# rhysnewell/Lorikeet

Hardware: AMD Instinct MI355X
Metric: PairHMM cell-updates/s (GCUPS) (higher is better)
Workload: dtype f64; 1 GPU; config2 x 1024 regions per GPU: 128 reads x 8 haps, R=150, H=300; regions_per_gpu=1024, seed=1000, env=PHMM_REGION_OWN_QUEUE=0 in this process only

## Files before the change

lorikeet_amd/csrc/phmm_chain_kernels.hip:

```cpp
#include "phmm_device.hpp"

namespace phmm {

namespace {

#ifndef PHMM_CHAIN_L
#define PHMM_CHAIN_L 16
#endif
constexpr int CL = PHMM_CHAIN_L;
#ifndef PHMM_RING
#define PHMM_RING 256
#endif
constexpr int RING = PHMM_RING;
constexpr int RING_SLOTS = RING + 4 + 1;
constexpr int CHAIN_META = CHAIN_MAX_READS + 8;
constexpr uint32_t X_PAD = 0x100u;
constexpr uint32_t X_NONE = 0x102u;
constexpr int LEAD = CL - 1;

__device__ __forceinline__ double from_left_inject(double v, double inject, bool group_head) {
    constexpr int ctrl = CL == 16 ? 0x111 : 0x138;
    int lo = __builtin_amdgcn_update_dpp(__double2loint(inject), __double2loint(v), ctrl, 0xf, 0xf, false);
    int hi = __builtin_amdgcn_update_dpp(__double2hiint(inject), __double2hiint(v), ctrl, 0xf, 0xf, false);
    if constexpr (CL == 32) {
        lo = group_head ? __double2loint(inject) : lo;
        hi = group_head ? __double2hiint(inject) : hi;
    }
    return __hiloint2double(hi, lo);
}

__device__ __forceinline__ RowConst row_bytes_one_go(const ForwardParams &p, uint32_t x, uint32_t q, uint32_t q_prev, uint32_t iq,
                                                     uint32_t dq, uint32_t dq_prev, uint32_t g, uint32_t g_next, bool first,
                                                     bool last) {
    const uint32_t mx = max(iq, dq), mn = min(iq, dq);
    const double mi = p.eps[iq], ii = p.eps[g], mm = p.mm[((mx * (mx + 1)) >> 1) + mn];
    const double e_g_next = p.eps[g_next], e_q_prev = p.eps[q_prev], e_dq_prev = p.eps[dq_prev];
    const double inv_om = p.inv_om[g], ratio_mis = p.ratio_mis[q];
    RowConst n;
    n.dd = ii;
    const double im = 1.0 - ii;
    const double im_next = last ? 1.0 : 1.0 - e_g_next;
    const double pm_prev = first ? 1.0 : 1.0 - e_q_prev;
    n.mm = mm * pm_prev;
    n.bI = mi * im_next * pm_prev;
    n.gI = ii * (im_next * inv_om);
    n.dDp = first ? 1.0 : e_dq_prev * im * pm_prev;
    n.pm = 1.0;
    n.px = (x == 'N') ? 1.0 : ratio_mis;
    n.x = x;
    n.pad0 = 0;
    n.pad1 = 0.0;
    return n;
}

template <int K>
__device__ __forceinline__ void chain_fallback(const ForwardParams &p, const ChainItem &it, RowConst *ring, int lane,
                                               int grp, int l, const HapCols<K> &hc, int H, bool hv, int a, int Nh) {
    const uint32_t reg = it.region;
    for (uint32_t r = it.read_begin; r < it.read_end; ++r) {
        const uint32_t ro = p.read_off[r];
        const int R = (int)(p.read_off[r + 1] - ro);
        bool z = false;
        for (int row = lane; row < R; row += WAVE) z |= row_blocks_prescale(p, ro + row);
        const bool scaled = __ballot(z) == 0ull;
        const bool staged = R + 1 <= RING;
        lds_wave_sync();
        if (staged) {
            if (lane == 0) ring[0] = neutral_row();
            for (int row = lane; row < R; row += WAVE) ring[row + 1] = make_row(p, ro, row, R, scaled);
        }
        lds_wave_sync();
        const double scale0 = (scaled && R > 0) ? 1.0 - p.eps[p.gcp[ro]] : 1.0;
        const double fin = (scaled && R > 0) ? 1.0 - p.eps[p.base_q[ro + R - 1]] : 1.0;
        const double c0 = p.initial_condition / (double)H * scale0;
        const bool group_head = (CL == 32) && (lane == 32);
        double s = staged ? sweep_general<CL, K>(LdsView{ring}, R, l, group_head, hc, H, c0, scaled, fin)
                          : sweep_general<CL, K>(GlobalRowView{p, ro, R, scaled}, R, l, group_head, hc, H, c0, scaled, fin);
#pragma unroll
        for (int off = CL / 2; off > 0; off >>= 1) s += __shfl_xor(s, off, WAVE);
        if (l == 0 && hv) {
            const double v = log10(s) - p.initial_condition_log10;
            p.out[p.out_off[reg] + (uint64_t)(r - p.region_read_off[reg]) * (uint64_t)Nh + a] = v;
            if (const uint32_t sb = status_bits(v)) atomicOr(p.status, sb);
        }
    }
    (void)grp;
}

template <int K>
__device__ __forceinline__ void chain_fallback_streams(const ForwardParams &p, uint32_t reg, uint32_t r_begin, int n_mine,
                                                       int n_iter, int lane, int l, const HapCols<K> &hc, int H, bool hv,
                                                       int a, int Nh) {
    const uint64_t group_bits = 0xffffull << (lane & ~15);
    for (int i = 0; i < n_iter; ++i) {
        const bool valid = i < n_mine;
        const uint32_t r = r_begin + (uint32_t)i;
        const uint32_t ro = valid ? p.read_off[r] : 0u;
        const int R = valid ? (int)(p.read_off[r + 1] - ro) : 0;
        bool z = false;
        for (int row = l; row < R; row += 16) z |= row_blocks_prescale(p, ro + row);
        const bool scaled = (__ballot(z) & group_bits) == 0ull;
        const double scale0 = (scaled && R > 0) ? 1.0 - p.eps[p.gcp[ro]] : 1.0;
        const double fin = (scaled && R > 0) ? 1.0 - p.eps[p.base_q[ro + R - 1]] : 1.0;
        const double c0 = p.initial_condition / (double)H * scale0;
        double s = sweep_general<16, K>(GlobalRowView{p, ro, R, scaled}, R, l, false, hc, H, c0, scaled, fin);
#pragma unroll
        for (int off = 8; off > 0; off >>= 1) s += __shfl_xor(s, off, WAVE);
        if (l == 0 && hv && valid) {
            const double v = log10(s) - p.initial_condition_log10;
            p.out[p.out_off[reg] + (uint64_t)(r - p.region_read_off[reg]) * (uint64_t)Nh + a] = v;
            if (const uint32_t sb = status_bits(v)) atomicOr(p.status, sb);
        }
    }
}

}

template <int CLT, int K, int MODE = CHAIN_PLAIN>
__device__ __forceinline__ void chain_body(const ForwardParams &p, const ChainItem it, unsigned char *smem, const ChainItemX *x = nullptr,
                                           double *park = nullptr) {
    static_assert(CLT == CL, "one lanes-per-pair value per compilation unit");
    static_assert(MODE == CHAIN_PLAIN || CL == 16, "prefix sharing: 16 lanes per pair");
    const int col0 = MODE == CHAIN_SUFFIX ? (int)x->mask_or_col0 : 0;
    const uint32_t park_rows = MODE == CHAIN_PLAIN ? 0u : 16u * x->park_rows16;
    const uint32_t park_mask = MODE == CHAIN_PARK ? (uint32_t)x->mask_or_col0 : 0u;
    const int lane = threadIdx.x;
    const int grp = lane / CL, l = lane % CL;
    const bool group_head = (CL == 32) && (lane == 32);
    const uint32_t reg = it.region;
    const int n_chain = (int)(it.read_end - it.read_begin);
    const uint32_t h0 = p.region_hap_off[reg];
    const int Nh = (int)(p.region_hap_off[reg + 1] - h0);
    const int S = (CL == 16) ? (int)it.streams : 1;
    const int GS = (WAVE / CL) / S;
    const int sid = grp / GS;
    const int a = MODE == CHAIN_PLAIN ? (int)it.quad * GS + grp % GS : (int)x->hap[grp & 3];
    const bool hv = a < Nh;
    const int n_sub = (n_chain + S - 1) / S;
    const int TPS = (RING / 4) / S;
    const int NM = RING / S - 1;
    auto n_of = [&](int s) { return max(0, min(n_sub, n_chain - s * n_sub)); };
    const int n_mine = n_of(sid);
    uint32_t ho = 0;
    int H = 0;
    if (hv) {
        ho = p.hap_off[h0 + a];
        H = (int)(p.hap_off[h0 + a + 1] - ho);
    }
    RowConst *ring = reinterpret_cast<RowConst *>(smem);
    uint32_t *roff = reinterpret_cast<uint32_t *>(ring + RING_SLOTS);
    uint32_t *stot = roff + CHAIN_META;

    HapCols<K> hc;
    bool lane_n = false;
#pragma unroll
    for (int w = 0; w < HapCols<K>::W; ++w) hc.y[w] = 0u;
#pragma unroll
    for (int k = 0; k < K; ++k) {
        const int col = col0 + l * K + k;
        uint32_t y = col < H ? (uint32_t)p.hap_bases[ho + col] : X_PAD;
        const bool is_n = (y == 'N');
        lane_n |= is_n;
        hc.set(k, y);
    }

    const uint32_t rb = it.read_begin;
    const uint32_t byte0 = p.read_off[rb];
    const uint32_t bytes = p.read_off[it.read_end] - byte0;
    const bool z = chain_blocks_prescale(p, byte0, bytes, lane);
    if ((__ballot(z) | __ballot(lane_n)) != 0ull) {
        if constexpr (MODE == CHAIN_SUFFIX) {
            for (uint32_t r = rb + (uint32_t)l; r < it.read_end && hv; r += CL)
                p.out[p.out_off[reg] + (uint64_t)(r - p.region_read_off[reg]) * (uint64_t)Nh + a] = __longlong_as_double(0x7ff8000000000000ll);
            if (lane == 0) atomicOr(p.status, STATUS_RESCUE);
            return;
        }
        if (S == 1)
            chain_fallback<K>(p, it, ring, lane, grp, l, hc, H, hv, a, Nh);
        else if constexpr (CL == 16)
            chain_fallback_streams<K>(p, reg, rb + (uint32_t)(sid * n_sub), n_mine, n_sub, lane, l, hc, H, hv, a, Nh);
        return;
    }
    {
        const int sj = lane / n_sub, ij = lane % n_sub;
        uint32_t len = lane < n_chain ? p.read_off[rb + lane + 1] - p.read_off[rb + lane] + 2u : 0u;
        uint32_t incl = len;
#pragma unroll
        for (int off = 1; off < WAVE; off <<= 1) {
            const uint32_t v = __shfl_up(incl, off, WAVE);
            if (lane >= off) incl += v;
        }
        const uint32_t before = __shfl(incl, max(sj * n_sub - 1, 0), WAVE);
        const int cb = sj * (n_sub + 1);
        if (lane < 4) stot[lane] = 0u;
        if (lane < n_chain) {
            roff[cb + ij] = p.read_off[rb + lane];
            if (ij + 1 == n_of(sj)) {
                roff[cb + ij + 1] = p.read_off[rb + lane + 1];
                stot[sj] = incl - (sj > 0 ? before : 0u);
            }
        }
        if (lane == 0) ring[RING_SLOTS - 1] = neutral_row();
    }
    lds_wave_sync();
    const int S_max = (int)max(max(stot[0], stot[1]), max(stot[2], stot[3]));
    const double c_unit = ldexp(1.0, 1010);

    uint32_t pb_x = 0, pb_q = 0, pb_qp = 0, pb_i = 0, pb_d = 0, pb_dp = 0, pb_g = 0, pb_gn = 0;
    double pb_bM = 0.0, pb_bD = 0.0;
    int p_Q = 0;
    const bool producer = lane < S * TPS;
    const int ps = producer ? lane / TPS : 0, pj = lane % TPS;
    const int pcb = ps * (n_sub + 1), pn = n_of(ps);
    int p_lo = 0, p_row = pj - LEAD - TPS;
    p_Q = pj - TPS;
    uint32_t p_ro = pn > 0 ? roff[pcb] : 0u;
    int p_R = pn > 0 ? (int)(roff[pcb + 1] - p_ro) : 0;
    auto advance = [&]() {
        p_row += TPS;
        p_Q += TPS;
        while (p_lo < pn && p_row >= p_R + 2) {
            p_row -= p_R + 2;
            ++p_lo;
            if (p_lo < pn) {
                p_ro = roff[pcb + p_lo];
                p_R = (int)(roff[pcb + p_lo + 1] - p_ro);
            }
        }
    };
    auto issue = [&]() {
        advance();
        const int row = p_row, R = p_R;
        const uint32_t ro = p_ro;
        if constexpr (MODE == CHAIN_SUFFIX) {
            if (producer && p_lo < pn && row >= 0 && (uint32_t)p_Q < park_rows) {
                const double *at = park + 2 * ((size_t)x->park_row0 + (size_t)p_Q);
                pb_bM = at[0];
                pb_bD = at[1];
            }
        }
        const bool live = producer && p_lo < pn && row >= 0 && R > 0;
        const uint32_t at = live ? ro + (uint32_t)min(row, R - 1) : byte0;
        const uint32_t at_prev = live ? ro + (uint32_t)max(min(row, R) - 1, 0) : byte0;
        const uint32_t at_next = live ? ro + (uint32_t)min(row + 1, R - 1) : byte0;
        const uint32_t at_g = (live && row > R && p_lo + 1 < pn) ? ro + (uint32_t)R : at;
        pb_x = p.read_bases[at];
        pb_q = p.base_q[at];
        pb_i = p.ins_q[at];
        pb_d = p.del_q[at];
        pb_g = p.gcp[at_g];
        pb_qp = p.base_q[at_prev];
        pb_dp = p.del_q[at_prev];
        pb_gn = p.gcp[at_next];
    };
    auto finish = [&](int Q0) {
        const int Q = Q0 + pj;
        const int lo = p_lo, row = p_row, R = p_R;
        constexpr bool ONE_GO = K <= 21;
        RowConst plain;
        double pm_last = 0.0;
        if constexpr (ONE_GO) {
            plain = row_bytes_one_go(p, pb_x, pb_q, pb_qp, pb_i, pb_d, pb_dp, pb_g, pb_gn, row == 0, row + 1 >= R);
            pm_last = 1.0 - p.eps[pb_qp];
        }
        RowConst n;
        if (lo < pn && row >= 0) {
            if (row < R) {
                if constexpr (ONE_GO) n = plain;
                else n = make_row_bytes(p, pb_x, pb_q, pb_qp, pb_i, pb_d, pb_dp, pb_g, pb_gn, row == 0, row + 1 >= R, true);
            } else if (row == R) {
                if constexpr (!ONE_GO) pm_last = 1.0 - p.eps[pb_qp];
                n.mm = pm_last; n.bI = n.mm; n.gI = 1.0; n.dDp = 0.0; n.dd = 1.0; n.pm = 1.0; n.px = 1.0;
                n.x = X_PAD; n.pad0 = (uint32_t)lo; n.pad1 = 0.0;
            } else {
                n.mm = 0.0; n.bI = 0.0; n.gI = 0.0; n.dDp = 0.0; n.dd = 1.0; n.pm = 0.0; n.px = 0.0;
                n.x = X_NONE; n.pad0 = 0;
                double e_first;
                if constexpr (ONE_GO) e_first = plain.dd;
                else e_first = p.eps[pb_g];
                n.pad1 = c_unit * (lo + 1 < pn ? 1.0 - e_first : 1.0);
            }
            if constexpr (MODE == CHAIN_SUFFIX) {
                n.pm = pb_bM;
                n.pad1 = pb_bD;
            }
        } else {
            n = neutral_row();
        }
        if (producer) {
            const int slot = ps * (NM + 2) + (Q & NM);
            ring[slot] = n;
            if ((Q & NM) == 0) ring[slot + NM + 1] = n;
        }
    };
    const double c0 = c_unit * (n_mine > 0 ? 1.0 - p.eps[p.gcp[roff[sid * (n_sub + 1)]]] : 1.0);
    issue();
    finish(0);
    issue();
    finish(TPS);
    issue();
    finish(2 * TPS);
    lds_wave_sync();
    issue();

    double Mp[K], Ip[K], Dp[K];
#pragma unroll
    for (int k = 0; k < K; ++k) {
        Mp[k] = 0.0;
        Ip[k] = 0.0;
        Dp[k] = c0;
    }
    double aM, aI, aD, bM = 0.0, bI = 0.0, bD = c0;
    const int edge_lane = (H > col0 ? H - 1 - col0 : 0) / K, edge_k = (H > col0 ? H - 1 - col0 : 0) % K;
    const bool last_lane = (l == edge_lane);
    const uint32_t sum_code = last_lane ? X_PAD : 0xffffffffu;
    const double log10_scale = log10(c_unit) + log10((double)H);
    auto emit = [&](const RowConst &c) {
        {
            if (last_lane && c.x == X_PAD && hv) {
                const uint32_t r = rb + (uint32_t)(sid * n_sub) + c.pad0;
                int ek = edge_k;
                asm volatile("" : "+v"(ek));
                double sum = 0.0;
#pragma unroll
                for (int k = 0; k < K; ++k)
                    if (k == ek) sum = (Dp[k] + Mp[k]) + Ip[k];
                const double v = log10(sum) - log10_scale;
                p.out[p.out_off[reg] + (uint64_t)(r - p.region_read_off[reg]) * (uint64_t)Nh + a] = v;
                if (const uint32_t sb = status_bits(v)) atomicOr(p.status, sb);
            }
        }
    };

    int q = LEAD - l;
    const int my_ring = sid * (NM + 2);
    const uint32_t my_rows = (uint32_t)(uintptr_t)(ring + my_ring);
    RowConst cA = lds_row(ring, my_ring + (q & NM)), cB;
    int q1 = q + 1;
    const int T = (S_max + CL - 1 + 1) & ~1;
    bool park_lane = false;
    double2 *park_at = nullptr;
    if constexpr (MODE == CHAIN_PARK) {
        park_lane = grp == 0 && ((park_mask >> l) & 1u) != 0u && hv && (uint32_t)(q + T) <= park_rows;
        const int b = __popc(park_mask & ((1u << l) - 1u));
        park_at = reinterpret_cast<double2 *>(park) + ((size_t)x->park_row0 + (size_t)b * park_rows + (size_t)q);
    }
    const int phase = (int)((blockIdx.x * 2654435761u) >> 26) & (TPS - 2);
    for (int t0 = 0, t1 = min(T, TPS - phase), tick = 0; t0 < T; t0 = t1, t1 = min(T, t1 + TPS), ++tick) {
        if (tick >= 1) {
            finish(TPS * tick + 2 * TPS);
            lds_wave_sync();
            issue();
        }
        for (int t = t0; t < t1; t += 2) {
            uint32_t pair_at;
            asm("v_mad_u32_u24 %0, %1, %2, %3" : "=v"(pair_at) : "v"((uint32_t)(q1 & NM)), "s"((uint32_t)sizeof(RowConst)), "v"(my_rows));
            cB = lds_row_at(pair_at, 0);
            if constexpr (MODE == CHAIN_SUFFIX) {
                aI = from_left_inject(Ip[K - 1], fma(bM, cA.bI, bI * cA.gI), group_head);
                aM = from_left_inject(Mp[K - 1], cA.pm, group_head);
            } else {
                aM = from_left<CL>(Mp[K - 1], group_head);
                aI = from_left<CL>(Ip[K - 1], group_head);
            }
            aD = from_left_inject(Dp[K - 1], cA.pad1, group_head);
            row_update<K, ROW_FAST_EXEC>(Mp, Ip, Dp, bM, bI, bD, aM, aD, cA, hc, 1.0);
            if constexpr (MODE == CHAIN_PARK)
                if (park_lane) park_at[0] = make_double2(Mp[K - 1], Dp[K - 1]);
            if (__ballot(cA.x == sum_code) != 0ull) emit(cA);
            cA = lds_row_at(pair_at, 1);
            if constexpr (MODE == CHAIN_SUFFIX) {
                bI = from_left_inject(Ip[K - 1], fma(aM, cB.bI, aI * cB.gI), group_head);
                bM = from_left_inject(Mp[K - 1], cB.pm, group_head);
            } else {
                bM = from_left<CL>(Mp[K - 1], group_head);
                bI = from_left<CL>(Ip[K - 1], group_head);
            }
            bD = from_left_inject(Dp[K - 1], cB.pad1, group_head);
            row_update<K, ROW_FAST_EXEC>(Mp, Ip, Dp, aM, aI, aD, bM, bD, cB, hc, 1.0);
            if constexpr (MODE == CHAIN_PARK) {
                if (park_lane) park_at[1] = make_double2(Mp[K - 1], Dp[K - 1]);
                park_at += 2;
            }
            if (__ballot(cB.x == sum_code) != 0ull) emit(cB);
            q1 += 2;
        }
    }
}


#define PHMM_CHAIN_K_LIST(X) \
    X(2) X(3) X(4) X(5) X(6) X(7) X(8) X(9) X(10) X(11) X(12) X(13) X(14) X(15) X(16) X(17) X(18) X(19) X(20) X(21) X(22) \
    X(23) X(24) X(25)

template <int CLT, int KLO, int KHI>
__global__ __launch_bounds__(WAVE, 2) void phmm_forward_chain(const ChainParams cp) {
    extern __shared__ __attribute__((aligned(16))) unsigned char smem[];
    const ChainItem it = cp.items[blockIdx.x];
    switch (__builtin_amdgcn_readfirstlane((int)it.k)) {
#define PHMM_CASE(KK)                                                  \
    case KK:                                                           \
        if constexpr (KK >= KLO && KK <= KHI) chain_body<CLT, KK>(cp.f, it, smem); \
        break;
        PHMM_CHAIN_K_LIST(PHMM_CASE)
#undef PHMM_CASE
        default:
            break;
    }
}

template <int CLT, int K>
__global__ __launch_bounds__(WAVE, 2) void phmm_forward_chain_k(const ChainParams cp) {
    extern __shared__ __attribute__((aligned(16))) unsigned char smem[];
    chain_body<CLT, K>(cp.f, cp.items[blockIdx.x], smem);
}

#define PHMM_CHAIN_CAT2(a, b) a##b
#define PHMM_CHAIN_CAT(a, b) PHMM_CHAIN_CAT2(a, b)
#define PHMM_CHAIN_LAUNCH PHMM_CHAIN_CAT(launch_chain_L, PHMM_CHAIN_L)

hipError_t PHMM_CHAIN_LAUNCH(int single_k, const ChainParams &cp, hipStream_t stream) {
    const size_t lds = (size_t)RING_SLOTS * sizeof(RowConst) + (CHAIN_META + 4) * sizeof(uint32_t);
#define PHMM_CASE(KK)                                                                                     \
    if (single_k == KK) {                                                                                 \
        hipLaunchKernelGGL((phmm_forward_chain_k<CL, KK>), dim3(cp.n_items), dim3(WAVE), lds, stream, cp); \
        return hipGetLastError();                                                                         \
    }
    PHMM_CHAIN_K_LIST(PHMM_CASE)
#undef PHMM_CASE
#define PHMM_RANGE(R, LO, HI)                                                                                       \
    if (single_k == -(R + 1)) {                                                                                     \
        hipLaunchKernelGGL((phmm_forward_chain<CL, LO, HI>), dim3(cp.n_items), dim3(WAVE), lds, stream, cp);        \
        return hipGetLastError();                                                                                   \
    }
    PHMM_CHAIN_RANGES(PHMM_RANGE)
#undef PHMM_RANGE
    return hipErrorInvalidValue;
}

#if PHMM_CHAIN_L == 16
hipError_t launch_chain_L32(int single_k, const ChainParams &cp, hipStream_t stream);
hipError_t launch_chain_L64(int single_k, const ChainParams &cp, hipStream_t stream);
int chain_max_k() { return 25; }
hipError_t launch_chain(int L, int single_k, const ChainParams &cp, hipStream_t stream) {
    if (!cp.n_items) return hipSuccess;
    return L == 16 ? launch_chain_L16(single_k, cp, stream) : L == 32 ? launch_chain_L32(single_k, cp, stream)
         : L == 64 ? launch_chain_L64(single_k, cp, stream) : hipErrorInvalidValue;
}
#endif

}
```

lorikeet_amd/csrc/phmm_device.hpp:

```cpp
#pragma once
#include "phmm_internal.hpp"

#include <type_traits>

#ifndef PHMM_SDWA_MIN_K
#define PHMM_SDWA_MIN_K 21
#endif
#ifndef PHMM_CND_MAX_K
#define PHMM_CND_MAX_K 13
#endif
#ifndef PHMM_TWO_WAVE_MAX_K
#define PHMM_TWO_WAVE_MAX_K 25
#endif

namespace phmm {

__device__ __forceinline__ int dpp_row_shr1(int v) {
    return __builtin_amdgcn_update_dpp(0, v, 0x111, 0xf, 0xf, true);
}
__device__ __forceinline__ int dpp_wave_shr1(int v) {
    return __builtin_amdgcn_update_dpp(0, v, 0x138, 0xf, 0xf, true);
}

template <int L>
__device__ __forceinline__ double from_left(double v, bool group_head) {
    int lo = __double2loint(v), hi = __double2hiint(v);
    if constexpr (L == 16) {
        lo = dpp_row_shr1(lo);
        hi = dpp_row_shr1(hi);
    } else {
        lo = dpp_wave_shr1(lo);
        hi = dpp_wave_shr1(hi);
        if constexpr (L == 32) {
            lo = group_head ? 0 : lo;
            hi = group_head ? 0 : hi;
        }
    }
    return __hiloint2double(hi, lo);
}

struct alignas(8) RowConst {
    double mm, bI, gI, dDp, dd, pm, px;
    uint32_t x, pad0;
    double pad1;
};
static_assert(sizeof(RowConst) == 72, "LDS row record");

__device__ __forceinline__ RowConst lds_row(const RowConst *rows, int idx) {
    return *reinterpret_cast<const RowConst *>(reinterpret_cast<const unsigned char *>(rows) +
                                               __mul24(idx, (int)sizeof(RowConst)));
}

__device__ __forceinline__ RowConst lds_row_at(uint32_t at, int skip) {
    RowConst r;
#if defined(__HIP_DEVICE_COMPILE__)
    typedef const __attribute__((address_space(3))) unsigned long long *LdsU64;
    const LdsU64 w = (LdsU64)(uintptr_t)at + skip * (int)(sizeof(RowConst) / 8);
    unsigned long long v[sizeof(RowConst) / 8];
#pragma unroll
    for (int i = 0; i < (int)(sizeof(RowConst) / 8) - 1; ++i) v[i] = w[i];
    v[8] = w[8];
    __builtin_memcpy(&r, v, sizeof r);
#else
    (void)at;
    (void)skip;
    r = RowConst{};
#endif
    return r;
}

struct LdsView {
    const RowConst *rows;
    __device__ __forceinline__ RowConst load(int idx) const { return lds_row(rows, idx); }
};

template <int K, class F>
__device__ __forceinline__ void static_for_down(F &&f) {
    if constexpr (K > 0) {
        f(std::integral_constant<int, K - 1>{});
        static_for_down<K - 1>(f);
    }
}

template <int K>
struct HapCols {
    static constexpr int W = (K + 1) / 2;
    uint32_t y[W];
    __device__ __forceinline__ uint16_t base(int k) const { return (uint16_t)(y[k >> 1] >> (16 * (k & 1))); }
    __device__ __forceinline__ void set(int k, uint32_t yv) { y[k >> 1] |= yv << (16 * (k & 1)); }
};

enum : int { ROW_GENERAL = 0, ROW_FAST_CND = 1, ROW_FAST_EXEC = 2, ROW_FAST_EXEC_PRED = 3 };

template <int K, int MODE>
__device__ __forceinline__ void row_update(double (&Mp)[K], double (&Ip)[K], double (&Dp)[K], const double plM,
                                           const double plI, const double plD, const double lM, const double lD,
                                           const RowConst &c, const HapCols<K> &hc, const double imx,
                                           const uint64_t live = ~0ull) {
    const uint16_t x16 = (uint16_t)c.x;
    if constexpr (MODE == ROW_FAST_EXEC || MODE == ROW_FAST_EXEC_PRED) {
        const uint64_t restore = (MODE == ROW_FAST_EXEC) ? ~0ull : live;
        constexpr bool packed = K > PHMM_SDWA_MIN_K;
        constexpr bool pred = MODE == ROW_FAST_EXEC_PRED;
        uint64_t mask;
        {
            constexpr int k = K - 1;
            const uint32_t y = packed ? hc.y[k >> 1] : (uint32_t)hc.base(k);
            if constexpr (packed && (k & 1))
                asm volatile("v_cmp_ne_u32_sdwa %0, %1, %2 src0_sel:DWORD src1_sel:WORD_1" : "=s"(mask) : "v"(c.x), "v"(y));
            else if constexpr (packed)
                asm volatile("v_cmp_ne_u32_sdwa %0, %1, %2 src0_sel:DWORD src1_sel:WORD_0" : "=s"(mask) : "v"(c.x), "v"(y));
            else
                asm volatile("v_cmp_ne_u32_e64 %0, %1, %2" : "=s"(mask) : "v"(c.x), "v"(y));
        }
        Ip[K - 1] = fma(Mp[K - 1], c.bI, Ip[K - 1] * c.gI);
        static_for_down<K>([&](auto kc) {
            constexpr int k = decltype(kc)::value;
            constexpr int km1 = k > 0 ? k - 1 : 0;
            const uint32_t yn = packed ? hc.y[km1 >> 1] : (uint32_t)hc.base(km1);
            uint64_t next;
#define PHMM_CELL(CMP, RESTORE)                                                                                      \
    asm volatile("v_fma_f64 %[M], %[Dl], %[dDp], %[Il]\n\t"                                                        \
                 "v_fma_f64 %[M], %[Ml], %[mm], %[M]\n\t"                                                          \
                 "s_mov_b64 exec, %[mk]\n\t"                                                                       \
                 "v_mul_f64 %[M], %[px], %[M]\n\t"                                                                 \
                 "s_mov_b64 exec, " RESTORE "\n\t"                                                                 \
                 CMP "\n\t"                                                                                      \
                 "v_mul_f64 %[Il], %[Il], %[gI]\n\t"                                                               \
                 "v_fma_f64 %[Il], %[Ml], %[bI], %[Il]"                                                             \
                 : [M] "=&v"(Mp[k]), [Il] "+v"(Ip[km1]), [mn] "=&s"(next)                                           \
                 : [Dl] "v"(Dp[km1]), [dDp] "v"(c.dDp), [Ml] "v"(Mp[km1]), [mm] "v"(c.mm), [x] "v"(c.x), [y] "v"(yn), \
                   [px] "v"(c.px), [gI] "v"(c.gI), [bI] "v"(c.bI), [live] "s"(restore), [mk] "s"(mask))
            if constexpr (k > 0 && pred && packed && (km1 & 1)) {
                PHMM_CELL("v_cmp_ne_u32_sdwa %[mn], %[x], %[y] src0_sel:DWORD src1_sel:WORD_1", "%[live]");
            } else if constexpr (k > 0 && pred && packed) {
                PHMM_CELL("v_cmp_ne_u32_sdwa %[mn], %[x], %[y] src0_sel:DWORD src1_sel:WORD_0", "%[live]");
            } else if constexpr (k > 0 && pred) {
                PHMM_CELL("v_cmp_ne_u32_e64 %[mn], %[x], %[y]", "%[live]");
            } else if constexpr (k > 0 && packed && (km1 & 1)) {
                PHMM_CELL("v_cmp_ne_u32_sdwa %[mn], %[x], %[y] src0_sel:DWORD src1_sel:WORD_1", "-1");
            } else if constexpr (k > 0 && packed) {
                PHMM_CELL("v_cmp_ne_u32_sdwa %[mn], %[x], %[y] src0_sel:DWORD src1_sel:WORD_0", "-1");
            } else if constexpr (k > 0) {
                PHMM_CELL("v_cmp_ne_u32_e64 %[mn], %[x], %[y]", "-1");
#undef PHMM_CELL
            } else {
                (void)yn;
                double m = fma(plM, c.mm, fma(plD, c.dDp, plI));
                asm volatile("s_mov_b64 exec, %2\n\t"
                             "v_mul_f64 %0, %1, %0\n\t"
                             "s_mov_b64 exec, %3"
                             : "+v"(m)
                             : "v"(c.px), "s"(mask), "s"(restore));
                Mp[0] = m;
                next = 0;
            }
            mask = next;
        });
        double leftM = lM, leftD = lD;
#pragma unroll
        for (int k = 0; k < K; ++k) {
            Dp[k] = fma(leftD, c.dd, leftM);
            leftM = Mp[k];
            leftD = Dp[k];
        }
        return;
    }
    static_for_down<K>([&](auto kc) {
        constexpr int k = decltype(kc)::value;
        Ip[k] = fma(Mp[k], c.bI, Ip[k] * c.gI);
        constexpr int km1 = k > 0 ? k - 1 : 0;
        const double dM = k > 0 ? Mp[km1] : plM;
        const double dI = k > 0 ? Ip[km1] : plI;
        const double dD = k > 0 ? Dp[km1] : plD;
        double t = fma(dD, c.dDp, dI);
        if constexpr (MODE == ROW_GENERAL) t *= imx;
        const double a = fma(dM, c.mm, t);
        const uint16_t yb = hc.base(k);
        const double prior = (x16 == yb || (MODE == ROW_GENERAL && yb == (uint16_t)'N')) ? c.pm : c.px;
        Mp[k] = prior * a;
    });
    double leftM = lM, leftD = lD;
#pragma unroll
    for (int k = 0; k < K; ++k) {
        Dp[k] = fma(leftD, c.dd, leftM);
        leftM = Mp[k];
        leftD = Dp[k];
    }
}


template <int L, int K, int STEADY = ROW_FAST_EXEC>
__device__ __forceinline__ double sweep_fast(const LdsView &lds, const int R, const int l, const bool group_head,
                                             const HapCols<K> &hc, const int H, const double c0, const double fin) {
    double Mp[K], Ip[K], Dp[K];
#pragma unroll
    for (int k = 0; k < K; ++k) {
        Mp[k] = 0.0;
        Ip[k] = 0.0;
        Dp[k] = c0;
    }
    double aM, aI, aD, bM = 0.0, bI = 0.0, bD = c0;
    int row = -l;
    RowConst cA = lds.load(max(row + 1, 0)), cB;
    int t = 0;
    for (; t + 1 < R; t += 2) {
        cB = lds.load(max(row + 2, 0));
        aM = from_left<L>(Mp[K - 1], group_head);
        aI = from_left<L>(Ip[K - 1], group_head);
        aD = from_left<L>(Dp[K - 1], group_head);
        row_update<K, STEADY>(Mp, Ip, Dp, bM, bI, bD, aM, aD, cA, hc, 1.0);
        cA = lds.load(max(row + 3, 0));
        bM = from_left<L>(Mp[K - 1], group_head);
        bI = from_left<L>(Ip[K - 1], group_head);
        bD = from_left<L>(Dp[K - 1], group_head);
        row_update<K, STEADY>(Mp, Ip, Dp, aM, aI, aD, bM, bD, cB, hc, 1.0);
        row += 2;
    }
    RowConst cur = cA;
    double plM = bM, plI = bI, plD = bD;
    if (t < R) {
        const RowConst nxt = lds.load(max(row + 2, 0));
        const double lM = from_left<L>(Mp[K - 1], group_head);
        const double lI = from_left<L>(Ip[K - 1], group_head);
        const double lD = from_left<L>(Dp[K - 1], group_head);
        row_update<K, STEADY>(Mp, Ip, Dp, plM, plI, plD, lM, lD, cur, hc, 1.0);
        plM = lM;
        plI = lI;
        plD = lD;
        ++row;
        cur = nxt;
    }
    for (int d = 0; d < L - 1; ++d) {
        const RowConst nxt = lds.load(max(min(row + 2, R), 0));
        const double lM = from_left<L>(Mp[K - 1], group_head);
        const double lI = from_left<L>(Ip[K - 1], group_head);
        const double lD = from_left<L>(Dp[K - 1], group_head);
        const uint64_t live = __ballot(row < R);
        if (row < R)
            row_update<K, STEADY == ROW_FAST_CND ? ROW_FAST_CND : ROW_FAST_EXEC_PRED>(Mp, Ip, Dp, plM, plI, plD, lM, lD, cur,
                                                                                     hc, 1.0, live);
        plM = lM;
        plI = lI;
        plD = lD;
        ++row;
        cur = nxt;
    }
    double s = 0.0;
#pragma unroll
    for (int k = 0; k < K; ++k)
        if (l * K + k < H) s += fma(Mp[k], fin, Ip[k]);
    return s;
}

template <int L, int K, class RowView>
__device__ __forceinline__ double sweep_general(const RowView &lds, const int R, const int l, const bool group_head,
                                             const HapCols<K> &hc, const int H, const double c0, const bool scaled,
                                             const double fin) {
    double Mp[K], Ip[K], Dp[K];
#pragma unroll
    for (int k = 0; k < K; ++k) {
        Mp[k] = 0.0;
        Ip[k] = 0.0;
        Dp[k] = c0;
    }
    double plM = 0.0, plI = 0.0, plD = c0;
    int row = -l;
    for (int t = 0; t < R + L - 1; ++t) {
        const RowConst cur = lds.load(max(min(row + 1, R), 0));
        const double lM = from_left<L>(Mp[K - 1], group_head);
        const double lI = from_left<L>(Ip[K - 1], group_head);
        const double lD = from_left<L>(Dp[K - 1], group_head);
        const double imx = scaled ? 1.0 : 1.0 - cur.dd;
        if (row < R) row_update<K, ROW_GENERAL>(Mp, Ip, Dp, plM, plI, plD, lM, lD, cur, hc, imx);
        plM = lM;
        plI = lI;
        plD = lD;
        ++row;
    }
    double s = 0.0;
#pragma unroll
    for (int k = 0; k < K; ++k)
        if (l * K + k < H) s += fma(Mp[k], fin, Ip[k]);
    return s;
}


__device__ __forceinline__ RowConst make_row_bytes(const ForwardParams &p, uint32_t x, uint32_t q, uint32_t q_prev,
                                                   uint32_t iq, uint32_t dq, uint32_t dq_prev, uint32_t g,
                                                   uint32_t g_next, bool first, bool last, bool scaled) {
    const double mi = p.eps[iq], ii = p.eps[g];
    const uint32_t mx = max(iq, dq), mn = min(iq, dq);
    const double mm = p.mm[((mx * (mx + 1)) >> 1) + mn];
    RowConst n;
    n.dd = ii;
    if (scaled) {
        const double im = 1.0 - ii;
        const double im_next = last ? 1.0 : 1.0 - p.eps[g_next];
        const double pm_prev = first ? 1.0 : 1.0 - p.eps[q_prev];
        n.mm = mm * pm_prev;
        n.bI = mi * im_next * pm_prev;
        n.gI = ii * (im_next * p.inv_om[g]);
        n.dDp = first ? 1.0 : p.eps[dq_prev] * im * pm_prev;
        n.pm = 1.0;
        n.px = (x == 'N') ? 1.0 : p.ratio_mis[q];
    } else {
        const double pm = 1.0 - p.eps[q];
        const double px = (x == 'N') ? pm : p.eps_mis[q];
        n.mm = mm;
        n.bI = mi;
        n.gI = ii;
        n.dDp = first ? 1.0 : p.eps[dq_prev];
        n.pm = pm;
        n.px = px;
    }
    n.x = x;
    n.pad0 = 0;
    n.pad1 = 0.0;
    return n;
}

__device__ __forceinline__ RowConst make_row(const ForwardParams &p, uint32_t ro, int row, int R, bool scaled) {
    const bool first = row == 0, last = row + 1 >= R;
    return make_row_bytes(p, p.read_bases[ro + row], p.base_q[ro + row], first ? 0u : (uint32_t)p.base_q[ro + row - 1],
                          p.ins_q[ro + row], p.del_q[ro + row], first ? 0u : (uint32_t)p.del_q[ro + row - 1],
                          p.gcp[ro + row], last ? 0u : (uint32_t)p.gcp[ro + row + 1], first, last, scaled);
}

__device__ __forceinline__ RowConst neutral_row();

struct GlobalRowView {
    const ForwardParams &p;
    uint32_t ro;
    int R;
    bool scaled;
    __device__ __forceinline__ RowConst load(int idx) const {
        return idx == 0 ? neutral_row() : make_row(p, ro, idx - 1, R, scaled);
    }
};

__device__ __forceinline__ bool row_blocks_prescale(const ForwardParams &p, uint32_t byte) {
    return p.gcp[byte] == 0 || p.base_q[byte] == 0;
}

__device__ __forceinline__ uint32_t zero_byte_in(uint32_t w) { return (w - 0x01010101u) & ~w & 0x80808080u; }
__device__ __forceinline__ bool chain_blocks_prescale(const ForwardParams &p, uint32_t byte0, uint32_t bytes, int lane) {
    if (bytes == 0u) return false;
    const uint8_t *g = p.gcp + byte0, *b = p.base_q + byte0;
    const uint32_t hg = min((uint32_t)(-(uintptr_t)g & 15u), bytes), hb = min((uint32_t)(-(uintptr_t)b & 15u), bytes);
    const uint32_t nv = (bytes - max(hg, hb)) >> 4;
    const uint32_t eg = lane < 16 ? (uint32_t)lane : hg + 16u * nv + (uint32_t)(lane - 16);
    const uint32_t eb = lane < 16 ? (uint32_t)lane : hb + 16u * nv + (uint32_t)(lane - 16);
    const bool in_g = lane < 16 ? eg < hg : eg < bytes, in_b = lane < 16 ? eb < hb : eb < bytes;
    const uint32_t edge_g = g[in_g ? eg : 0u], edge_b = b[in_b ? eb : 0u];
    const uint4 *G = reinterpret_cast<const uint4 *>(g + hg), *B = reinterpret_cast<const uint4 *>(b + hb);
    uint32_t found = 0u;
    constexpr int SCAN_DEPTH = 4;
#pragma clang loop unroll(disable) vectorize(disable) interleave(disable)
    for (uint32_t v0 = 0; v0 < nv; v0 += SCAN_DEPTH * WAVE) {
        uint4 vg[SCAN_DEPTH], vb[SCAN_DEPTH];
#pragma unroll
        for (int j = 0; j < SCAN_DEPTH; ++j) {
            const uint32_t v = min(v0 + (uint32_t)(j * WAVE + lane), nv - 1u);
            vg[j] = G[v];
            vb[j] = B[v];
        }
#pragma unroll
        for (int j = 0; j < SCAN_DEPTH; ++j)
            found |= zero_byte_in(vg[j].x) | zero_byte_in(vg[j].y) | zero_byte_in(vg[j].z) | zero_byte_in(vg[j].w) |
                     zero_byte_in(vb[j].x) | zero_byte_in(vb[j].y) | zero_byte_in(vb[j].z) | zero_byte_in(vb[j].w);
    }
    return found != 0u || edge_g == 0u || edge_b == 0u;
}

__device__ __forceinline__ RowConst neutral_row() {
    RowConst n;
    n.mm = 0.0; n.bI = 0.0; n.gI = 1.0; n.dDp = 0.0; n.dd = 1.0; n.pm = 0.0; n.px = 0.0;
    n.x = 0; n.pad0 = 0; n.pad1 = 0.0;
    return n;
}

__device__ __forceinline__ void lds_wave_sync() {
    __builtin_amdgcn_fence(__ATOMIC_RELEASE, "wavefront");
    __builtin_amdgcn_wave_barrier();
    __builtin_amdgcn_fence(__ATOMIC_ACQUIRE, "wavefront");
}

template <int L, int K>
__device__ __forceinline__ void forward_read(const ForwardParams &p, const uint32_t r, const int quad_begin, const int quad_step,
                                             const bool cnd_select, unsigned char *smem_wave, double *coherent_out = nullptr) {
    constexpr int G = WAVE / L;
    const int lane = threadIdx.x & (WAVE - 1);
    const int grp = lane / L, l = lane % L;
    const uint32_t reg = p.read_region[r];
    const uint32_t ro = p.read_off[r];
    const int R = (int)(p.read_off[r + 1] - ro);
    const uint32_t h0 = p.region_hap_off[reg];
    const int Nh = (int)(p.region_hap_off[reg + 1] - h0);
    double *out_row = p.out + p.out_off[reg] + (uint64_t)(r - p.region_read_off[reg]) * (uint64_t)Nh;

    RowConst *srow = reinterpret_cast<RowConst *>(smem_wave);
    bool lane_zero_gcp = false;
    for (int row = lane; row < R; row += WAVE) lane_zero_gcp |= row_blocks_prescale(p, ro + row);
    const bool scaled = __ballot(lane_zero_gcp) == 0ull;
    if (lane == 0) srow[0] = neutral_row();
    for (int row = lane; row < R; row += WAVE) srow[row + 1] = make_row(p, ro, row, R, scaled);
    const double scale0 = (scaled && R > 0) ? 1.0 - p.eps[p.gcp[ro]] : 1.0;
    const double fin = (scaled && R > 0) ? 1.0 - p.eps[p.base_q[ro + R - 1]] : 1.0;
    lds_wave_sync();
    const LdsView lds{srow};
    const bool group_head = (L == 32) && (lane == 32);

    const int nquads = (Nh + G - 1) / G;
    for (int quad = quad_begin; quad < nquads; quad += quad_step) {
        const int a = quad * G + grp;
        const bool hv = a < Nh;
        uint32_t ho = 0;
        int H = 0;
        if (hv) {
            ho = p.hap_off[h0 + a];
            H = (int)(p.hap_off[h0 + a + 1] - ho);
        }
        HapCols<K> hc;
        bool lane_n = false;
#pragma unroll
        for (int w = 0; w < HapCols<K>::W; ++w) hc.y[w] = 0u;
#pragma unroll
        for (int k = 0; k < K; ++k) {
            const int col = l * K + k;
            const uint32_t y = (col < H) ? (uint32_t)p.hap_bases[ho + col] : 0u;
            const bool is_n = (y == 'N');
            lane_n |= is_n;
            hc.set(k, y);
        }
        const double c0 = p.initial_condition / (double)H * scale0;
        double s;
        if (scaled && __ballot(lane_n) == 0ull) {
            if constexpr (K <= PHMM_CND_MAX_K) {
                s = cnd_select ? sweep_fast<L, K, ROW_FAST_CND>(lds, R, l, group_head, hc, H, c0, fin)
                               : sweep_fast<L, K>(lds, R, l, group_head, hc, H, c0, fin);
            } else {
                s = sweep_fast<L, K>(lds, R, l, group_head, hc, H, c0, fin);
            }
        } else {
            s = sweep_general<L, K>(lds, R, l, group_head, hc, H, c0, scaled, fin);
        }
#pragma unroll
        for (int off = L / 2; off > 0; off >>= 1) s += __shfl_xor(s, off, WAVE);
        if (l == 0 && hv) {
            const double v = log10(s) - p.initial_condition_log10;
            if (coherent_out) __hip_atomic_store(&coherent_out[a], v, __ATOMIC_RELAXED, __HIP_MEMORY_SCOPE_AGENT);
            else out_row[a] = v;
            if (const uint32_t sb = status_bits(v)) atomicOr(p.status, sb);
        }
    }
}

}
```

Baseline: 4671 GCUPS.

## Group cell updates into multi-cell inline asm blocks and split pad1 LDS load

Adds a new row_update mode that processes up to three haplotype cells per inline-asm block. It batches the exec-mask switches for the mismatch multiply and interleaves the compares with the FMA chains, aiming to cut scalar exec toggles and expose more ILP. The mode is used for K up to the SDWA threshold. The pad1 field is now read by a separate volatile LDS load issued before the next row load, with lds_row_at no longer loading the last word. This shortens the dependency on that field for the D injection. The hand-scheduled asm constrains the compiler's register allocation and scheduling, and zeroing the last word changes the semantics of lds_row_at for every other caller.

```diff
diff --git a/lorikeet_amd/csrc/phmm_chain_kernels.hip b/lorikeet_amd/csrc/phmm_chain_kernels.hip
--- a/lorikeet_amd/csrc/phmm_chain_kernels.hip
+++ b/lorikeet_amd/csrc/phmm_chain_kernels.hip
@@ -335,7 +335,8 @@
     int q = LEAD - l;
     const int my_ring = sid * (NM + 2);
     const uint32_t my_rows = (uint32_t)(uintptr_t)(ring + my_ring);
-    RowConst cA = lds_row(ring, my_ring + (q & NM)), cB;
+    uint32_t pair_at = my_rows + (uint32_t)((q - 1) & NM) * (uint32_t)sizeof(RowConst);
+    RowConst cA = lds_row_at(pair_at, 1), cB;
     int q1 = q + 1;
     const int T = (S_max + CL - 1 + 1) & ~1;
     bool park_lane = false;
@@ -345,6 +346,7 @@
         const int b = __popc(park_mask & ((1u << l) - 1u));
         park_at = reinterpret_cast<double2 *>(park) + ((size_t)x->park_row0 + (size_t)b * park_rows + (size_t)q);
     }
+    constexpr int STEP = K <= PHMM_SDWA_MIN_K ? ROW_FAST_EXEC_GROUPED : ROW_FAST_EXEC;
     const int phase = (int)((blockIdx.x * 2654435761u) >> 26) & (TPS - 2);
     for (int t0 = 0, t1 = min(T, TPS - phase), tick = 0; t0 < T; t0 = t1, t1 = min(T, t1 + TPS), ++tick) {
         if (tick >= 1) {
@@ -353,7 +355,7 @@
             issue();
         }
         for (int t = t0; t < t1; t += 2) {
-            uint32_t pair_at;
+            const double padA = lds_pad1_at(pair_at, 1);
             asm("v_mad_u32_u24 %0, %1, %2, %3" : "=v"(pair_at) : "v"((uint32_t)(q1 & NM)), "s"((uint32_t)sizeof(RowConst)), "v"(my_rows));
             cB = lds_row_at(pair_at, 0);
             if constexpr (MODE == CHAIN_SUFFIX) {
@@ -363,11 +365,12 @@
                 aM = from_left<CL>(Mp[K - 1], group_head);
                 aI = from_left<CL>(Ip[K - 1], group_head);
             }
-            aD = from_left_inject(Dp[K - 1], cA.pad1, group_head);
-            row_update<K, ROW_FAST_EXEC>(Mp, Ip, Dp, bM, bI, bD, aM, aD, cA, hc, 1.0);
+            aD = from_left_inject(Dp[K - 1], padA, group_head);
+            row_update<K, STEP>(Mp, Ip, Dp, bM, bI, bD, aM, aD, cA, hc, 1.0);
             if constexpr (MODE == CHAIN_PARK)
                 if (park_lane) park_at[0] = make_double2(Mp[K - 1], Dp[K - 1]);
             if (__ballot(cA.x == sum_code) != 0ull) emit(cA);
+            const double padB = lds_pad1_at(pair_at, 0);
             cA = lds_row_at(pair_at, 1);
             if constexpr (MODE == CHAIN_SUFFIX) {
                 bI = from_left_inject(Ip[K - 1], fma(aM, cB.bI, aI * cB.gI), group_head);
@@ -376,8 +379,8 @@
                 bM = from_left<CL>(Mp[K - 1], group_head);
                 bI = from_left<CL>(Ip[K - 1], group_head);
             }
-            bD = from_left_inject(Dp[K - 1], cB.pad1, group_head);
-            row_update<K, ROW_FAST_EXEC>(Mp, Ip, Dp, aM, aI, aD, bM, bD, cB, hc, 1.0);
+            bD = from_left_inject(Dp[K - 1], padB, group_head);
+            row_update<K, STEP>(Mp, Ip, Dp, aM, aI, aD, bM, bD, cB, hc, 1.0);
             if constexpr (MODE == CHAIN_PARK) {
                 if (park_lane) park_at[1] = make_double2(Mp[K - 1], Dp[K - 1]);
                 park_at += 2;
diff --git a/lorikeet_amd/csrc/phmm_device.hpp b/lorikeet_amd/csrc/phmm_device.hpp
--- a/lorikeet_amd/csrc/phmm_device.hpp
+++ b/lorikeet_amd/csrc/phmm_device.hpp
@@ -59,7 +59,7 @@
     unsigned long long v[sizeof(RowConst) / 8];
 #pragma unroll
     for (int i = 0; i < (int)(sizeof(RowConst) / 8) - 1; ++i) v[i] = w[i];
-    v[8] = w[8];
+    v[8] = 0ull;
     __builtin_memcpy(&r, v, sizeof r);
 #else
     (void)at;
@@ -69,6 +69,18 @@
     return r;
 }
 
+__device__ __forceinline__ double lds_pad1_at(uint32_t at, int skip) {
+#if defined(__HIP_DEVICE_COMPILE__)
+    typedef const volatile __attribute__((address_space(3))) unsigned long long *LdsU64;
+    const LdsU64 w = (LdsU64)(uintptr_t)at + skip * (int)(sizeof(RowConst) / 8);
+    return __longlong_as_double((long long)w[8]);
+#else
+    (void)at;
+    (void)skip;
+    return 0.0;
+#endif
+}
+
 struct LdsView {
     const RowConst *rows;
     __device__ __forceinline__ RowConst load(int idx) const { return lds_row(rows, idx); }
@@ -90,7 +102,7 @@
     __device__ __forceinline__ void set(int k, uint32_t yv) { y[k >> 1] |= yv << (16 * (k & 1)); }
 };
 
-enum : int { ROW_GENERAL = 0, ROW_FAST_CND = 1, ROW_FAST_EXEC = 2, ROW_FAST_EXEC_PRED = 3 };
+enum : int { ROW_GENERAL = 0, ROW_FAST_CND = 1, ROW_FAST_EXEC = 2, ROW_FAST_EXEC_PRED = 3, ROW_FAST_EXEC_GROUPED = 4 };
 
 template <int K, int MODE>
 __device__ __forceinline__ void row_update(double (&Mp)[K], double (&Ip)[K], double (&Dp)[K], const double plM,
@@ -98,6 +110,74 @@
                                            const RowConst &c, const HapCols<K> &hc, const double imx,
                                            const uint64_t live = ~0ull) {
     const uint16_t x16 = (uint16_t)c.x;
+    if constexpr (MODE == ROW_FAST_EXEC_GROUPED) {
+        static_assert(K <= PHMM_SDWA_MIN_K, "grouped cells compare unpacked haplotype bases");
+#define PHMM_G_C(m, y) "v_cmp_ne_u32_e64 %[" m "], %[x], %[" y "]\n\t"
+#define PHMM_G_M(M, D, I, Ml) "v_fma_f64 %[" M "], %[" D "], %[dDp], %[" I "]\n\tv_fma_f64 %[" M "], %[" Ml "], %[mm], %[" M "]\n\t"
+#define PHMM_G_I(I, Ml) "v_mul_f64 %[" I "], %[" I "], %[gI]\n\tv_fma_f64 %[" I "], %[" Ml "], %[bI], %[" I "]\n\t"
+#define PHMM_G_X(m, M) "s_mov_b64 exec, %[" m "]\n\tv_mul_f64 %[" M "], %[px], %[" M "]\n\t"
+#define PHMM_G_ALL "s_mov_b64 exec, -1\n\t"
+#define PHMM_G_CONST [dDp] "v"(c.dDp), [mm] "v"(c.mm), [x] "v"(c.x), [px] "v"(c.px), [gI] "v"(c.gI), [bI] "v"(c.bI), [mk] "s"(mask)
+        uint64_t mask;
+        asm volatile("v_cmp_ne_u32_e64 %0, %1, %2" : "=s"(mask) : "v"(c.x), "v"((uint32_t)hc.base(K - 1)));
+        asm volatile(PHMM_G_I("I", "M") : [I] "+v"(Ip[K - 1]) : [M] "v"(Mp[K - 1]), [gI] "v"(c.gI), [bI] "v"(c.bI));
+        static_for_down<K>([&](auto kc) {
+            constexpr int k = decltype(kc)::value;
+            constexpr int n = (K - 1 - k) % 3 != 0 ? 0 : k >= 3 ? 3 : k;
+            constexpr int k1 = k > 1 ? k - 1 : 0, k2 = k > 2 ? k - 2 : 0, k3 = k > 3 ? k - 3 : 0;
+            uint64_t next = 0, mb, mc;
+            (void)next, (void)mb, (void)mc, (void)k1, (void)k2, (void)k3;
+            if constexpr (n == 3) {
+                const uint32_t yb = (uint32_t)hc.base(k1), yc = (uint32_t)hc.base(k2), yd = (uint32_t)hc.base(k3);
+                asm volatile(PHMM_G_C("mb", "yb") PHMM_G_M("Ma", "Db", "Ib", "Mb") PHMM_G_I("Ib", "Mb")
+                             PHMM_G_C("mc", "yc") PHMM_G_M("Mb", "Dc", "Ic", "Mc") PHMM_G_I("Ic", "Mc")
+                             PHMM_G_M("Mc", "Dd", "Id", "Md")
+                             PHMM_G_X("mk", "Ma") PHMM_G_X("mb", "Mb") PHMM_G_X("mc", "Mc") PHMM_G_ALL
+                             PHMM_G_C("mn", "yd") PHMM_G_I("Id", "Md")
+                             : [Ma] "=&v"(Mp[k]), [Mb] "+v"(Mp[k1]), [Mc] "+v"(Mp[k2]), [Ib] "+v"(Ip[k1]), [Ic] "+v"(Ip[k2]),
+                               [Id] "+v"(Ip[k3]), [mn] "=&s"(next), [mb] "=&s"(mb), [mc] "=&s"(mc)
+                             : [Db] "v"(Dp[k1]), [Dc] "v"(Dp[k2]), [Dd] "v"(Dp[k3]), [Md] "v"(Mp[k3]), [yb] "v"(yb), [yc] "v"(yc),
+                               [yd] "v"(yd), PHMM_G_CONST);
+                mask = next;
+            } else if constexpr (n == 2) {
+                const uint32_t yb = (uint32_t)hc.base(k1), yc = (uint32_t)hc.base(k2);
+                asm volatile(PHMM_G_C("mb", "yb") PHMM_G_M("Ma", "Db", "Ib", "Mb") PHMM_G_I("Ib", "Mb")
+                             PHMM_G_M("Mb", "Dc", "Ic", "Mc")
+                             PHMM_G_X("mk", "Ma") PHMM_G_X("mb", "Mb") PHMM_G_ALL
+                             PHMM_G_C("mn", "yc") PHMM_G_I("Ic", "Mc")
+                             : [Ma] "=&v"(Mp[k]), [Mb] "+v"(Mp[k1]), [Ib] "+v"(Ip[k1]), [Ic] "+v"(Ip[k2]), [mn] "=&s"(next),
+                               [mb] "=&s"(mb)
+                             : [Db] "v"(Dp[k1]), [Dc] "v"(Dp[k2]), [Mc] "v"(Mp[k2]), [yb] "v"(yb), [yc] "v"(yc), PHMM_G_CONST);
+                mask = next;
+            } else if constexpr (n == 1) {
+                const uint32_t yb = (uint32_t)hc.base(k1);
+                asm volatile(PHMM_G_M("Ma", "Db", "Ib", "Mb") PHMM_G_X("mk", "Ma") PHMM_G_ALL
+                             PHMM_G_C("mn", "yb") PHMM_G_I("Ib", "Mb")
+                             : [Ma] "=&v"(Mp[k]), [Ib] "+v"(Ip[k1]), [mn] "=&s"(next)
+                             : [Db] "v"(Dp[k1]), [Mb] "v"(Mp[k1]), [yb] "v"(yb), PHMM_G_CONST);
+                mask = next;
+            } else if constexpr (k == 0) {
+                double m;
+                asm(PHMM_G_M("M", "Dl", "Il", "Ml") : [M] "=&v"(m) : [Dl] "v"(plD), [dDp] "v"(c.dDp), [Il] "v"(plI), [Ml] "v"(plM), [mm] "v"(c.mm));
+                asm volatile(PHMM_G_X("mk", "M") PHMM_G_ALL : [M] "+v"(m) : [px] "v"(c.px), [mk] "s"(mask));
+                Mp[0] = m;
+            }
+        });
+#undef PHMM_G_C
+#undef PHMM_G_M
+#undef PHMM_G_I
+#undef PHMM_G_X
+#undef PHMM_G_ALL
+#undef PHMM_G_CONST
+        double leftM = lM, leftD = lD;
+#pragma unroll
+        for (int k = 0; k < K; ++k) {
+            Dp[k] = fma(leftD, c.dd, leftM);
+            leftM = Mp[k];
+            leftD = Dp[k];
+        }
+        return;
+    }
     if constexpr (MODE == ROW_FAST_EXEC || MODE == ROW_FAST_EXEC_PRED) {
         const uint64_t restore = (MODE == ROW_FAST_EXEC) ? ~0ull : live;
         constexpr bool packed = K > PHMM_SDWA_MIN_K;
```

After: 4727 GCUPS (median of 6 runs). +1.2%, better.
